# szy4017/DeepSense6G_TII

Hardware: AMD Instinct MI355X
Metric: training samples/sec (5-frame seq, bs=12 per GPU) (higher is better)
Workload: dtype f32; 1 GPU; BASELINE configs[2]: full camera+LiDAR+radar+GPS fusion, 5x(3+1+2)x256x256 + 2x2 GPS per sample, bs=12 per GPU, sigmoid focal loss, AdamW, train-mode BN, dropout 0.1; global_batch=12, seq_len=5, parallelism=dp1, ema=False, launch=eager, optimizer=AdamW after backward

## Files before the change

deepsense6g_tii_amd/csrc/igemm.hip:

```cpp
#include "common.h"
#include "gemm_plan.h"
#include <vector>

extern int g_ds6g_attn_fused128;
extern int g_ds6g_attn_merged_sum;
extern int g_ds6g_attn_percu;
extern int g_ds6g_attn_handover;
extern int g_wino_kb64;

#ifndef IGEMM_STAGES_FD
#define IGEMM_STAGES_FD 3
#endif
#ifndef IGEMM_STAGES_W
#define IGEMM_STAGES_W 2
#endif

GCLK_STORAGE(g_igemm_clk, g_igemm_wg, ds6g_igemm_clocks_read)

namespace {

enum { MODE_FWD = 0, MODE_DGRAD = 1, MODE_WGRAD = 2 };

struct IgemmParams {
    const float* a_src;
    const float* b_src;
    float* out;
    int N, H, W, C;
    int Ho, Wo, K;
    int R, S, stride, pad;
    int Mg, Ng, Kg;
    const float* bias;
    const float* residual;
    const float* mask_src;
    int relu;
    int accumulate;
    uint32_t drop_thr;
    float drop_scale;
    uint64_t seed;
    uint64_t seed_off;
    const uint64_t* salt;
    int k_per_split;
    size_t split_stride;
    int tiles_n;
    int nclass;
    double prof_flops;
    int wg_rows;
    int is_linear;
    int want_colsum;
    int xcd_splits;
    int h0, hstep, Hs, w0, wstep, Ws, r0, rstep, nr, s0, sstep, ns;
    unsigned a_bytes, b_bytes;
    int dbg;
};


template <int MODE, int BM, int BN, int EPI, int BK, int BF, int FAST>
__global__ __launch_bounds__(256) void igemm_kernel(const IgemmParams pin) {
    IgemmParams p = pin;
    if (EPI && p.drop_thr && p.salt) p.seed_off += *p.salt;
    GCLK_DECL(g_igemm_wg);
    if (MODE == MODE_DGRAD && pin.nclass > 1) {
        const int ph = blockIdx.y >> 1, pw = blockIdx.y & 1;
        p.h0 = ph;
        p.w0 = pw;
        p.r0 = (ph + p.pad) & 1;
        p.nr = p.r0 < p.R ? (p.R - p.r0 + 1) / 2 : 0;
        p.s0 = (pw + p.pad) & 1;
        p.ns = p.s0 < p.S ? (p.S - p.s0 + 1) / 2 : 0;
        p.Kg = p.nr * p.ns * p.K;
        if (p.ns == 0) p.ns = 1;
        if (p.Kg == 0 && p.accumulate) return;
    }
    constexpr int CH = BK / 4;
    constexpr int RPB = 16 / CH;
    constexpr int KH = BK / 2;
    constexpr int TM = BM / 64;
    constexpr int TN = BN / 64;
    constexpr int A_LD = BM * CH / 256;
    constexpr int B_LD = BN * CH / 256;
    constexpr bool A_KMAJOR = (MODE == MODE_WGRAD);
    constexpr bool B_KMAJOR = (MODE != MODE_FWD);
    __shared__ __attribute__((aligned(16))) float As0[BM * BK];
    __shared__ __attribute__((aligned(16))) float As1[BM * BK];
    __shared__ __attribute__((aligned(16))) float Bs0[BN * BK];
    __shared__ __attribute__((aligned(16))) float Bs1[BN * BK];
    constexpr int NS = (MODE == MODE_WGRAD) ? IGEMM_STAGES_W : (BK == 32 ? 2 : IGEMM_STAGES_FD);
    static_assert(NS >= 2 && NS <= 4, "2..4 LDS stages");
    __shared__ __attribute__((aligned(16))) float As2[NS >= 3 ? BM * BK : 4];
    __shared__ __attribute__((aligned(16))) float Bs2[NS >= 3 ? BN * BK : 4];
    __shared__ __attribute__((aligned(16))) float As3[NS >= 4 ? BM * BK : 4];
    __shared__ __attribute__((aligned(16))) float Bs3[NS >= 4 ? BN * BK : 4];

    const int tid = threadIdx.x;
    const int lane = tid & 63;
    const int wave = __builtin_amdgcn_readfirstlane(tid >> 6);
    const int wm = wave >> 1, wn = wave & 1;
    int wg, split = blockIdx.z;
    if (MODE == MODE_WGRAD && p.xcd_splits) {
        const int nwg = gridDim.x * gridDim.z, orig = blockIdx.x + gridDim.x * blockIdx.z;
        const int q = nwg >> 3, r = nwg & 7, xcd = orig & 7;
        const int lin = (xcd < r ? xcd * (q + 1) : r * (q + 1) + (xcd - r) * q) + (orig >> 3);
        split = lin / (int)gridDim.x;
        wg = lin - split * (int)gridDim.x;
    } else {
        const int nwg = gridDim.x, orig = blockIdx.x;
        const int q = nwg >> 3, r = nwg & 7, xcd = orig & 7;
        wg = (xcd < r ? xcd * (q + 1) : r * (q + 1) + (xcd - r) * q) + (orig >> 3);
    }
    const int tile_m = wg / p.tiles_n;
    const int tile_n = wg - tile_m * p.tiles_n;
    const int m0 = tile_m * BM, n0 = tile_n * BN;
    const int kbegin = (MODE == MODE_WGRAD) ? split * p.k_per_split : 0;
    const int kend = (MODE == MODE_WGRAD) ? min(p.Kg, kbegin + p.k_per_split) : p.Kg;
    const int nk = (kend - kbegin + BK - 1) / BK;

    const i32x4 a_rsrc = make_srd(p.a_src, p.a_bytes);
    const i32x4 b_rsrc = make_srd(p.b_src, p.b_bytes);

    unsigned a_base[A_LD];
    int a_y[A_LD], a_x[A_LD];
    int a_c[A_LD], a_r[A_LD], a_s[A_LD], a_k[A_LD];
    bool a_ok[A_LD];
#pragma unroll
    for (int i = 0; i < A_LD; ++i) {
        const int idx = tid + i * 256;
        if (MODE == MODE_FWD || MODE == MODE_DGRAD) {
            const int row = idx / CH;
            const int m = m0 + row;
            a_ok[i] = m < p.Mg;
            const int mm = a_ok[i] ? m : 0;
            const int cin = (MODE == MODE_FWD) ? p.C : p.K;
            const int kg = ((idx % CH) ^ ((row / RPB) & (CH - 1))) * 4;
            a_k[i] = kg;
            const int tap = kg / cin;
            a_c[i] = kg - tap * cin;
            const int nsx = (MODE == MODE_DGRAD) ? p.ns : p.S;
            a_r[i] = tap / nsx;
            a_s[i] = tap - a_r[i] * nsx;
            if (MODE == MODE_FWD) {
                int ow, t, oh, n;
                fast_divmod(mm, p.Wo, t, ow);
                fast_divmod(t, p.Ho, n, oh);
                a_y[i] = oh * p.stride - p.pad;
                a_x[i] = ow * p.stride - p.pad;
                a_base[i] = (unsigned)n * (unsigned)(p.H * p.W * p.C);
            } else {
                int ww, t, hh, n;
                fast_divmod(mm, p.Ws, t, ww);
                fast_divmod(t, p.Hs, n, hh);
                a_y[i] = p.h0 + hh * p.hstep + p.pad;
                a_x[i] = p.w0 + ww * p.wstep + p.pad;
                a_base[i] = (unsigned)n * (unsigned)(p.Ho * p.Wo * p.K);
            }
        } else {
            const int mc = idx % (BM / 4);
            a_ok[i] = (m0 + mc * 4) < p.Mg;
            a_k[i] = kbegin + idx / (BM / 4);
            a_base[i] = (unsigned)(m0 + mc * 4);
            a_y[i] = a_x[i] = a_c[i] = a_r[i] = a_s[i] = 0;
        }
    }
    unsigned b_base[B_LD];
    int b_r[B_LD], b_s[B_LD];
    int b_k[B_LD];
    int b_o[B_LD], b_t[B_LD];
    int b_n[B_LD];
    bool b_ok[B_LD];
#pragma unroll
    for (int i = 0; i < B_LD; ++i) {
        const int idx = tid + i * 256;
        b_r[i] = b_s[i] = b_o[i] = b_t[i] = b_n[i] = 0;
        if (MODE == MODE_FWD) {
            const int row = idx / CH;
            b_ok[i] = (n0 + row) < p.Ng;
            b_k[i] = ((idx % CH) ^ ((row / RPB) & (CH - 1))) * 4;
            b_base[i] = (unsigned)(n0 + row) * (unsigned)p.Kg;
        } else if (MODE == MODE_DGRAD) {
            b_ok[i] = (n0 + (idx % (BN / 4)) * 4) < p.Ng;
            const int kg = idx / (BN / 4);
            b_k[i] = kg;
            const int tap = kg / p.K;
            b_o[i] = kg - tap * p.K;
            b_t[i] = tap / p.ns;
            b_n[i] = tap - b_t[i] * p.ns;
            b_base[i] = (unsigned)(n0 + (idx % (BN / 4)) * 4);
        } else {
            const int ncol = n0 + (idx % (BN / 4)) * 4;
            b_ok[i] = ncol < p.Ng;
            const int nn = b_ok[i] ? ncol : 0;
            const int tap = nn / p.C;
            b_r[i] = tap / p.S;
            b_s[i] = tap - b_r[i] * p.S;
            b_base[i] = (unsigned)(nn - tap * p.C);
            const int pix = kbegin + idx / (BN / 4);
            b_k[i] = pix;
            const int pp = pix < p.Kg ? pix : 0;
            b_o[i] = pp % p.Wo;
            const int t = pp / p.Wo;
            b_t[i] = t % p.Ho;
            b_n[i] = t / p.Ho;
        }
    }

    [[maybe_unused]] int u_c0 = 0, u_r = 0, u_s = 0;
    [[maybe_unused]] unsigned u_kb = 0;
    [[maybe_unused]] int u_kpos = kbegin, u_n = 0, u_oh = 0, u_ow = 0;
    [[maybe_unused]] unsigned a_vo[A_LD], b_vo[B_LD];
    [[maybe_unused]] int a_kr[A_LD], b_kr[B_LD], b_ihl[B_LD], b_iwl[B_LD];
    [[maybe_unused]] i32x4 b_rsrc_f = b_rsrc;
    auto retap = [&]() {
#pragma unroll
        for (int i = 0; i < A_LD; ++i) {
            if (MODE == MODE_FWD) {
                const int ih = a_y[i] + u_r, iw = a_x[i] + u_s;
                const bool ok = a_ok[i] && (unsigned)ih < (unsigned)p.H && (unsigned)iw < (unsigned)p.W;
                a_vo[i] = ok ? (a_base[i] + (unsigned)((ih * p.W + iw) * p.C + a_c[i])) * 4u : OOB_OFF;
            } else if (MODE == MODE_DGRAD) {
                const int th = a_y[i] - (p.r0 + u_r * p.rstep), tw = a_x[i] - (p.s0 + u_s * p.sstep);
                int oh = th, ow = tw;
                bool okk = th >= 0 && tw >= 0;
                if (p.stride == 2) {
                    oh = th >> 1;
                    ow = tw >> 1;
                    okk = okk && !((th | tw) & 1);
                } else if (p.stride != 1) {
                    oh = th / p.stride;
                    ow = tw / p.stride;
                    okk = okk && (oh * p.stride == th) && (ow * p.stride == tw);
                }
                const bool ok = a_ok[i] && okk && oh < p.Ho && ow < p.Wo;
                a_vo[i] = ok ? (a_base[i] + (unsigned)((oh * p.Wo + ow) * p.K + a_c[i])) * 4u : OOB_OFF;
            }
        }
    };
    if (FAST) {
        if (MODE == MODE_FWD) {
            retap();
#pragma unroll
            for (int i = 0; i < B_LD; ++i) b_vo[i] = b_ok[i] ? (b_base[i] + (unsigned)b_k[i]) * 4u : OOB_OFF;
        } else if (MODE == MODE_DGRAD) {
            retap();
#pragma unroll
            for (int i = 0; i < B_LD; ++i)
                b_vo[i] = b_ok[i] ? (b_base[i] + (unsigned)(b_o[i] * (p.R * p.S) * p.C)) * 4u : OOB_OFF;
        } else {
            if (p.wg_rows == 0) {
                u_ow = kbegin % p.Wo;
                const int t = kbegin / p.Wo;
                u_oh = t % p.Ho;
                u_n = t / p.Ho;
            } else {
                const int t = kbegin / p.Wo;
                u_oh = t % p.Ho;
                u_n = t / p.Ho;
            }
            const int shift = (p.pad * p.W + p.pad) * p.C;
            b_rsrc_f = make_srd(p.b_src - shift, p.b_bytes + (unsigned)shift * 4u);
#pragma unroll
            for (int i = 0; i < A_LD; ++i) {
                a_kr[i] = (tid + i * 256) / (BM / 4);
                a_vo[i] = (a_base[i] + (unsigned)(a_kr[i] * p.K)) * 4u;
            }
#pragma unroll
            for (int i = 0; i < B_LD; ++i) {
                b_kr[i] = (tid + i * 256) / (BN / 4);
                const int dl_oh = p.wg_rows == 0 ? 0 : b_kr[i] / p.Wo;
                const int dl_ow = p.wg_rows == 0 ? b_kr[i] : b_kr[i] % p.Wo;
                b_ihl[i] = dl_oh * p.stride - p.pad + b_r[i];
                b_iwl[i] = dl_ow * p.stride - p.pad + b_s[i];
                b_vo[i] = (unsigned)((int)b_base[i] + (b_ihl[i] * p.W + b_iwl[i]) * p.C + shift) * 4u;
            }
        }
    }

    auto issue_tiles = [&](float* Ad, float* Bd) {
        if (FAST) {
            if (MODE == MODE_FWD || MODE == MODE_DGRAD) {
                const unsigned sa = (unsigned)u_c0 * 4u;
                unsigned sb;
                if (MODE == MODE_FWD) {
                    sb = u_kb;
                } else {
                    const int tapw = (p.r0 + u_r * p.rstep) * p.S + p.s0 + u_s * p.sstep;
                    sb = (unsigned)((u_c0 * (p.R * p.S) + tapw) * p.C) * 4u;
                }
#pragma unroll
                for (int i = 0; i < A_LD; ++i)
                    dma16(a_rsrc, lds_addr(Ad) + (unsigned)(i * 256 + wave * 64) * 16u, (p.dbg & 32) ? OOB_OFF : a_vo[i], sa);
#pragma unroll
                for (int i = 0; i < B_LD; ++i)
                    dma16(b_rsrc, lds_addr(Bd) + (unsigned)(i * 256 + wave * 64) * 16u, (p.dbg & 32) ? OOB_OFF : b_vo[i], sb);
                u_kb += BK * 4;
                u_c0 += BK;
                if (u_c0 == ((MODE == MODE_FWD) ? p.C : p.K)) {
                    u_c0 = 0;
                    if (++u_s == ((MODE == MODE_FWD) ? p.S : p.ns)) { u_s = 0; ++u_r; }
                    retap();
                }
            } else {
                const int rows_left = kend - u_kpos;
                const unsigned sa = (unsigned)(u_kpos * p.K) * 4u;
                const int ihu = u_oh * p.stride, iwu = u_ow * p.stride;
                const unsigned sb = (unsigned)(((u_n * p.H + ihu) * p.W + iwu) * p.C) * 4u;
#pragma unroll
                for (int i = 0; i < A_LD; ++i) {
                    const bool ok = a_ok[i] && a_kr[i] < rows_left && !(p.dbg & 32);
                    dma16(a_rsrc, lds_addr(Ad) + (unsigned)(i * 256 + wave * 64) * 16u, ok ? a_vo[i] : OOB_OFF, sa);
                }
#pragma unroll
                for (int i = 0; i < B_LD; ++i) {
                    const bool ok = b_ok[i] && b_kr[i] < rows_left && (unsigned)(ihu + b_ihl[i]) < (unsigned)p.H &&
                                    (unsigned)(iwu + b_iwl[i]) < (unsigned)p.W && !(p.dbg & 32);
                    dma16(b_rsrc_f, lds_addr(Bd) + (unsigned)(i * 256 + wave * 64) * 16u, ok ? b_vo[i] : OOB_OFF, sb);
                }
                u_kpos += BK;
                if (p.wg_rows == 0) {
                    u_ow += BK;
                    if (u_ow >= p.Wo) {
                        u_ow = 0;
                        if (++u_oh == p.Ho) { u_oh = 0; ++u_n; }
                    }
                } else {
                    u_oh += p.wg_rows;
                    if (u_oh >= p.Ho) { u_oh = 0; ++u_n; }
                }
            }
            return;
        }
#pragma unroll
        for (int i = 0; i < A_LD; ++i) {
            unsigned off;
            bool ok = a_ok[i] && a_k[i] < kend;
            if (MODE == MODE_FWD) {
                const int ih = a_y[i] + a_r[i], iw = a_x[i] + a_s[i];
                ok = ok && ih >= 0 && ih < p.H && iw >= 0 && iw < p.W;
                off = a_base[i] + (unsigned)((ih * p.W + iw) * p.C + a_c[i]);
            } else if (MODE == MODE_DGRAD) {
                const int th = a_y[i] - (p.r0 + a_r[i] * p.rstep), tw = a_x[i] - (p.s0 + a_s[i] * p.sstep);
                int oh = th, ow = tw;
                bool okk = th >= 0 && tw >= 0;
                if (p.stride == 2) {
                    oh = th >> 1;
                    ow = tw >> 1;
                    okk = okk && !((th | tw) & 1);
                } else if (p.stride != 1) {
                    oh = th / p.stride;
                    ow = tw / p.stride;
                    okk = okk && (oh * p.stride == th) && (ow * p.stride == tw);
                }
                ok = ok && okk && oh < p.Ho && ow < p.Wo;
                off = a_base[i] + (unsigned)((oh * p.Wo + ow) * p.K + a_c[i]);
            } else {
                off = a_base[i] + (unsigned)a_k[i] * (unsigned)p.K;
            }
            if (p.dbg & 32) ok = false;
            dma16(a_rsrc, lds_addr(Ad) + (unsigned)(i * 256 + wave * 64) * 16u, ok ? off * 4u : OOB_OFF, 0u);
            a_k[i] += BK;
            if (MODE != MODE_WGRAD) {
                const int cin = (MODE == MODE_FWD) ? p.C : p.K;
                a_c[i] += BK;
                const int nsx = (MODE == MODE_DGRAD) ? p.ns : p.S;
                while (a_c[i] >= cin) {
                    a_c[i] -= cin;
                    if (++a_s[i] == nsx) { a_s[i] = 0; ++a_r[i]; }
                }
            }
        }
#pragma unroll
        for (int i = 0; i < B_LD; ++i) {
            unsigned off;
            bool ok = b_ok[i] && b_k[i] < kend;
            if (MODE == MODE_FWD) {
                off = b_base[i] + (unsigned)b_k[i];
            } else if (MODE == MODE_DGRAD) {
                const int tap = (p.r0 + b_t[i] * p.rstep) * p.S + p.s0 + b_n[i] * p.sstep;
                off = b_base[i] + (unsigned)((b_o[i] * (p.R * p.S) + tap) * p.C);
                b_o[i] += BK;
                while (b_o[i] >= p.K) {
                    b_o[i] -= p.K;
                    if (++b_n[i] == p.ns) { b_n[i] = 0; ++b_t[i]; }
                }
            } else {
                const int ih = b_t[i] * p.stride - p.pad + b_r[i];
                const int iw = b_o[i] * p.stride - p.pad + b_s[i];
                ok = ok && ih >= 0 && ih < p.H && iw >= 0 && iw < p.W;
                off = b_base[i] + (unsigned)(((b_n[i] * p.H + ih) * p.W + iw) * p.C);
                b_o[i] += BK;
                while (b_o[i] >= p.Wo) {
                    b_o[i] -= p.Wo;
                    if (++b_t[i] == p.Ho) { b_t[i] = 0; ++b_n[i]; }
                }
            }
            if (p.dbg & 32) ok = false;
            dma16(b_rsrc, lds_addr(Bd) + (unsigned)(i * 256 + wave * 64) * 16u, ok ? off * 4u : OOB_OFF, 0u);
            b_k[i] += BK;
        }
    };

    f32x16 acc[TM][TN];
#pragma unroll
    for (int i = 0; i < TM; ++i)
#pragma unroll
        for (int j = 0; j < TN; ++j)
#pragma unroll
            for (int r = 0; r < 16; ++r) acc[i][j][r] = 0.f;

    const int a_row = wm * (BM / 2) + (lane & 31);
    const int b_row = wn * (BN / 2) + (lane & 31);
    const int khalf = lane >> 5;
    const int swz = ((lane & 31) / RPB) & (CH - 1);

    float csum = 0.f;
    const bool do_csum = (MODE == MODE_WGRAD) && p.want_colsum && tile_n == 0 && tid < BM;
    auto k_step = [&](const float* Ac, const float* Bc, float* An, float* Bn, int rem) {
        if (NS >= 3) {
            if (NS >= 4 && rem >= 2) asm volatile("s_waitcnt vmcnt(%0)" ::"n"(2 * (A_LD + B_LD)) : "memory");
            else if (rem >= 1) asm volatile("s_waitcnt vmcnt(%0)" ::"n"(A_LD + B_LD) : "memory");
            else asm volatile("s_waitcnt vmcnt(0)" ::: "memory");
            GCLK(g_igemm_clk, 4);
            if (!(p.dbg & 4)) __syncthreads();
            GCLK(g_igemm_clk, 5);
        }
        if (rem >= NS - 1 && !(p.dbg & 1)) issue_tiles(An, Bn);
        GCLK(g_igemm_clk, 2);
        if (MODE == MODE_WGRAD && do_csum) {
#pragma unroll
            for (int k = 0; k < BK; ++k) csum += Ac[k * BM + tid];
        }
        float af[TM][KH], bf[TN][KH];
#pragma unroll
        for (int i = 0; i < TM; ++i) {
            if (A_KMAJOR) {
#pragma unroll
                for (int kk = 0; kk < KH; ++kk) af[i][kk] = Ac[(khalf * KH + kk) * BM + a_row + i * 32];
            } else {
                const float* rp = &Ac[(a_row + i * 32) * BK];
#pragma unroll
                for (int c = 0; c < CH / 2; ++c) {
                    const f32x4 v = *reinterpret_cast<const f32x4*>(rp + (((khalf * (CH / 2) + c) ^ swz) << 2));
#pragma unroll
                    for (int e = 0; e < 4; ++e) af[i][4 * c + e] = v[e];
                }
            }
        }
#pragma unroll
        for (int j = 0; j < TN; ++j) {
            if (B_KMAJOR) {
#pragma unroll
                for (int kk = 0; kk < KH; ++kk) bf[j][kk] = Bc[(khalf * KH + kk) * BN + b_row + j * 32];
            } else {
                const float* rp = &Bc[(b_row + j * 32) * BK];
#pragma unroll
                for (int c = 0; c < CH / 2; ++c) {
                    const f32x4 v = *reinterpret_cast<const f32x4*>(rp + (((khalf * (CH / 2) + c) ^ swz) << 2));
#pragma unroll
                    for (int e = 0; e < 4; ++e) bf[j][4 * c + e] = v[e];
                }
            }
        }
        __builtin_amdgcn_sched_barrier(0);
        if (BF) {
            static_assert(!BF || BK % 16 == 0, "bf16 k-tiles are multiples of 16");
#pragma unroll
            for (int q = 0; q < BK / 16; ++q) {
                if (BF == 3) {
                    bf16x8 ah[TM], am[TM], al3[TM], bh[TN], bm[TN], bl3[TN];
#pragma unroll
                    for (int i = 0; i < TM; ++i) split3_bf16x8(&af[i][8 * q], ah[i], am[i], al3[i]);
#pragma unroll
                    for (int j = 0; j < TN; ++j) split3_bf16x8(&bf[j][8 * q], bh[j], bm[j], bl3[j]);
#pragma unroll
                    for (int i = 0; i < TM; ++i)
#pragma unroll
                        for (int j = 0; j < TN; ++j)
                            acc[i][j] = mfma_x6(ah[i], am[i], al3[i], bh[j], bm[j], bl3[j], acc[i][j]);
                    continue;
                }
                bf16x8 a8[TM], b8[TN], al[TM], bl[TN];
#pragma unroll
                for (int i = 0; i < TM; ++i) {
                    if (BF == 2) split_bf16x8(&af[i][8 * q], a8[i], al[i]);
                    else {
#pragma unroll
                        for (int e = 0; e < 8; ++e) a8[i][e] = (__bf16)af[i][8 * q + e];
                    }
                }
#pragma unroll
                for (int j = 0; j < TN; ++j) {
                    if (BF == 2) split_bf16x8(&bf[j][8 * q], b8[j], bl[j]);
                    else {
#pragma unroll
                        for (int e = 0; e < 8; ++e) b8[j][e] = (__bf16)bf[j][8 * q + e];
                    }
                }
                if (BF == 2) {
#pragma unroll
                    for (int i = 0; i < TM; ++i)
#pragma unroll
                        for (int j = 0; j < TN; ++j)
                            acc[i][j] = __builtin_amdgcn_mfma_f32_32x32x16_bf16(al[i], b8[j], acc[i][j], 0, 0, 0);
#pragma unroll
                    for (int i = 0; i < TM; ++i)
#pragma unroll
                        for (int j = 0; j < TN; ++j)
                            acc[i][j] = __builtin_amdgcn_mfma_f32_32x32x16_bf16(a8[i], bl[j], acc[i][j], 0, 0, 0);
                }
#pragma unroll
                for (int i = 0; i < TM; ++i)
#pragma unroll
                    for (int j = 0; j < TN; ++j)
                        acc[i][j] = __builtin_amdgcn_mfma_f32_32x32x16_bf16(a8[i], b8[j], acc[i][j], 0, 0, 0);
            }
        } else {
#pragma unroll
            for (int kk = 0; kk < BK / 2; ++kk) {
#pragma unroll
                for (int i = 0; i < TM; ++i)
#pragma unroll
                    for (int j = 0; j < TN; ++j)
                        acc[i][j] = __builtin_amdgcn_mfma_f32_32x32x2f32(af[i][kk], bf[j][kk], acc[i][j], 0, 0, 0);
            }
        }
        __builtin_amdgcn_sched_barrier(0);
        GCLK(g_igemm_clk, 3);
        GCLK_COUNT(g_igemm_clk, 15);
        if (NS == 2) {
            asm volatile("s_waitcnt vmcnt(0)" ::: "memory");
            GCLK(g_igemm_clk, 4);
            if (!(p.dbg & 4)) __syncthreads();
            GCLK(g_igemm_clk, 5);
        }
    };

    float* const Ast[4] = {As0, As1, As2, As3};
    float* const Bst[4] = {Bs0, Bs1, Bs2, Bs3};
    [[maybe_unused]] float bias_pre[TN];
    if (EPI) {
#pragma unroll
        for (int j = 0; j < TN; ++j) {
            const int col = n0 + wn * (BN / 2) + j * 32 + (lane & 31);
            bias_pre[j] = (p.bias && col < p.Ng) ? p.bias[col] : 0.f;
        }
    }
    GCLK(g_igemm_clk, 0);
#pragma unroll
    for (int u = 0; u < NS - 1; ++u)
        if (u < nk && !(p.dbg & 16)) issue_tiles(Ast[u], Bst[u]);
    if (NS == 2) {
        asm volatile("s_waitcnt vmcnt(0)" ::: "memory");
        __syncthreads();
    }
    GCLK(g_igemm_clk, 1);
    for (int kt0 = 0; kt0 < nk; kt0 += NS) {
#pragma unroll
        for (int u = 0; u < NS; ++u) {
            const int kt = kt0 + u;
            if (kt < nk) k_step(Ast[u], Bst[u], Ast[(u + NS - 1) % NS], Bst[(u + NS - 1) % NS], nk - 1 - kt);
        }
    }

    float* outp = p.out + ((MODE == MODE_WGRAD) ? (size_t)split * p.split_stride : (size_t)0);
    if (MODE == MODE_WGRAD && do_csum && m0 + tid < p.Mg) outp[(size_t)p.Mg * p.Ng + m0 + tid] = csum;
    if (EPI == 0) {
        const auto o_rsrc = __builtin_amdgcn_make_buffer_rsrc(outp, 0, (unsigned)p.Mg * (unsigned)p.Ng * 4u, 0x00020000);
        const unsigned rowbytes = (unsigned)p.Ng * 4u;
#pragma unroll
        for (int i = 0; i < TM; ++i) {
#pragma unroll
            for (int j = 0; j < TN; ++j) {
                const int col = n0 + wn * (BN / 2) + j * 32 + (lane & 31);
                const int row0 = m0 + wm * (BM / 2) + i * 32 + 4 * khalf;
                const unsigned base = (col < p.Ng && !((p.dbg & 8) && (i | j)))
                                          ? (unsigned)row0 * rowbytes + (unsigned)col * 4u
                                          : OOB_OFF;
#pragma unroll
                for (int r = 0; r < 16; ++r) {
                    const unsigned off = base + (unsigned)((r & 3) + 8 * (r >> 2)) * rowbytes;
                    float v = acc[i][j][r];
                    if (MODE != MODE_WGRAD && p.accumulate)
                        v += __uint_as_float(__builtin_amdgcn_raw_buffer_load_b32(o_rsrc, off, 0, 0));
                    __builtin_amdgcn_raw_buffer_store_b32(__float_as_uint(v), o_rsrc, off, 0, 0);
                }
            }
        }
        GCLK(g_igemm_clk, 6);
        GCLK_END(g_igemm_clk, g_igemm_wg);
        return;
    }
    if (!(MODE == MODE_DGRAD && p.hstep != 1)) {
        const unsigned nbytes = (unsigned)p.Mg * (unsigned)p.Ng * 4u;
        const auto o_rsrc = __builtin_amdgcn_make_buffer_rsrc(outp, 0, nbytes, 0x00020000);
        const auto m_rsrc = __builtin_amdgcn_make_buffer_rsrc(const_cast<float*>(p.mask_src ? p.mask_src : outp), 0, nbytes, 0x00020000);
        const auto r_rsrc = __builtin_amdgcn_make_buffer_rsrc(const_cast<float*>(p.residual ? p.residual : outp), 0, nbytes, 0x00020000);
        const unsigned rowbytes = (unsigned)p.Ng * 4u;
#pragma unroll
        for (int i = 0; i < TM; ++i) {
#pragma unroll
            for (int j = 0; j < TN; ++j) {
                const int col = n0 + wn * (BN / 2) + j * 32 + (lane & 31);
                const int row0 = m0 + wm * (BM / 2) + i * 32 + 4 * khalf;
                const bool cok = col < p.Ng;
                const float bias = bias_pre[j];
                const unsigned base = cok ? (unsigned)row0 * rowbytes + (unsigned)col * 4u : OOB_OFF;
                const unsigned e0 = (unsigned)row0 * (unsigned)p.Ng + (unsigned)col;
#pragma unroll
                for (int r = 0; r < 16; ++r) {
                    const unsigned dr = (unsigned)((r & 3) + 8 * (r >> 2));
                    const unsigned off = base + dr * rowbytes;
                    float v = acc[i][j][r] + bias;
                    if (p.relu == 1) v = fmaxf(v, 0.f);
                    if (p.mask_src) v = (__uint_as_float(__builtin_amdgcn_raw_buffer_load_b32(m_rsrc, off, 0, 0)) > 0.f) ? v : 0.f;
                    if (p.drop_thr)
                        v = ds6g_keep(p.seed, p.seed_off + (uint64_t)(e0 + dr * (unsigned)p.Ng), p.drop_thr) ? v * p.drop_scale : 0.f;
                    if (p.residual) v += __uint_as_float(__builtin_amdgcn_raw_buffer_load_b32(r_rsrc, off, 0, 0));
                    if (p.accumulate) v += __uint_as_float(__builtin_amdgcn_raw_buffer_load_b32(o_rsrc, off, 0, 0));
                    if (p.relu == 2) v = fmaxf(v, 0.f);
                    __builtin_amdgcn_raw_buffer_store_b32(__float_as_uint(v), o_rsrc, off, 0, 0);
                }
            }
        }
        GCLK(g_igemm_clk, 6);
        GCLK_END(g_igemm_clk, g_igemm_wg);
        return;
    }
#pragma unroll
    for (int i = 0; i < TM; ++i) {
#pragma unroll
        for (int j = 0; j < TN; ++j) {
            const int col = n0 + wn * (BN / 2) + j * 32 + (lane & 31);
            if (col >= p.Ng) continue;
#pragma unroll
            for (int r = 0; r < 16; ++r) {
                const int row = m0 + wm * (BM / 2) + i * 32 + (r & 3) + 8 * (r >> 2) + 4 * khalf;
                if (row >= p.Mg) continue;
                const int ww = row % p.Ws;
                const int t = row / p.Ws;
                const int hh = t % p.Hs;
                const size_t orow = ((size_t)(t / p.Hs) * p.H + p.h0 + hh * p.hstep) * p.W + p.w0 + ww * p.wstep;
                const size_t o = orow * p.Ng + col;
                float v = acc[i][j][r];
                if (p.accumulate) v += outp[o];
                outp[o] = v;
            }
        }
    }
    GCLK(g_igemm_clk, 6);
    GCLK_END(g_igemm_clk, g_igemm_wg);
}

constexpr int RED_COLS = 16, RED_LANES = 16;
__global__ __launch_bounds__(256) void splitk_reduce_kernel(const float* __restrict__ part, float* __restrict__ out,
                                                            long n4, float* __restrict__ out_b, long m4, int splits,
                                                            size_t stride, int accumulate, int accumulate_b) {
    __shared__ f32x4 red[RED_LANES][RED_COLS];
    const int col = threadIdx.x & (RED_COLS - 1), sl = threadIdx.x / RED_COLS;
    const long i = (long)blockIdx.x * RED_COLS + col;
    f32x4 s = {0.f, 0.f, 0.f, 0.f};
    if (i < n4 + m4)
        for (int k = sl; k < splits; k += RED_LANES) s += *reinterpret_cast<const f32x4*>(part + (size_t)k * stride + i * 4);
    red[sl][col] = s;
    __syncthreads();
    if (sl != 0 || i >= n4 + m4) return;
#pragma unroll
    for (int l = 1; l < RED_LANES; ++l) s += red[l][col];
    const bool is_b = i >= n4;
    f32x4* o = is_b ? reinterpret_cast<f32x4*>(out_b + (i - n4) * 4) : reinterpret_cast<f32x4*>(out + i * 4);
    if (is_b ? accumulate_b : accumulate) s += *o;
    *o = s;
}

static_assert(GEMM_ERR_ARG == DS6G_ERR_ARG && GEMM_ERR_WORKSPACE == DS6G_ERR_WORKSPACE && GEMM_OOB == OOB_OFF, "gemm_plan.h");

int g_last_variant = -1;

struct ProfRec { int variant; double flops; hipEvent_t e0, e1; };
std::vector<ProfRec>* g_prof = nullptr;
size_t g_prof_cap = 0;

GemmKnobs g_knobs;
GemmKnobs igemm_knobs() {
    static const bool env_read = [] {
        gemm_env("DS6G_WGRAD_TARGET_LIN", &g_knobs.wgrad_target_lin);
        gemm_env("DS6G_WGRAD_TARGET_CONV", &g_knobs.wgrad_target_conv);
        gemm_env("DS6G_WGRAD_XCD", &g_knobs.wgrad_xcd);
        return true;
    }();
    (void)env_read;
    GemmKnobs kn = g_knobs;
    kn.operand_mode = g_ds6g_bf16;
    return kn;
}

}

void* ds6g_prof_open(int variant, double flops, hipStream_t st) {
    if (!g_prof || g_prof->size() >= g_prof_cap) return nullptr;
    g_prof->push_back(ProfRec{});
    ProfRec* rec = &g_prof->back();
    rec->variant = variant;
    rec->flops = flops;
    (void)hipEventCreate(&rec->e0);
    (void)hipEventCreate(&rec->e1);
    (void)hipEventRecord(rec->e0, st);
    return rec;
}
void ds6g_prof_close(void* rec, hipStream_t st) {
    if (rec) (void)hipEventRecord(static_cast<ProfRec*>(rec)->e1, st);
}

int ds6g_internal_splitk_reduce(const float* ws, float* dw, long n4, float* dbias, long m4, int splits, size_t stride,
                                int accumulate, int accumulate_b, hipStream_t st) {
    hipLaunchKernelGGL(splitk_reduce_kernel, dim3(cdiv(n4 + m4, RED_COLS)), dim3(256), 0, st, ws, dw, n4, dbias, m4, splits,
                       stride, accumulate, accumulate_b);
    DS6G_LAUNCH_CHECK();
    return DS6G_OK;
}

GemmKnobs ds6g_internal_bgemm_knobs();

namespace {

int plan_params(const GemmProblem& q, GemmPlan& pl, IgemmParams& p) {
    if (const int rc = gemm_plan_params(q, igemm_knobs(), pl, p)) return rc;
    p.is_linear = q.op >= DS6G_GEMM_LINEAR_FWD && q.op <= DS6G_GEMM_LINEAR_WGRAD;
    if (pl.nclass > 1) p.prof_flops = 2.0 * p.Mg * p.Ng * (double)(p.R * p.S) * p.K;
    p.dbg = g_knobs.dbg;
    return DS6G_OK;
}

template <int MODE, int CODE>
void launch_igemm(const IgemmParams& p, const GemmPlan& pl, hipStream_t st) {
    constexpr int BF = CODE % 4, KW = CODE / 4 % 3, EPI = CODE / 12 % 2, TILE = CODE / 24;
    constexpr int BM = TILE == 2 ? 64 : 128, BN = TILE == 0 ? 128 : 64;
    if constexpr (!(MODE == MODE_WGRAD && KW == 2))
        hipLaunchKernelGGL((igemm_kernel<MODE, BM, BN, EPI, KW == 2 ? 32 : 16, BF, KW != 0>), dim3(pl.grid_x, pl.grid_y, pl.grid_z),
                           dim3(256), 0, st, p);
}

int run_igemm(const IgemmParams& p, const GemmPlan& pl, float* dw, float* dbias, int accumulate, hipStream_t st) {
    void* rec = ds6g_prof_open(pl.variant, p.prof_flops > 0 ? p.prof_flops : 2.0 * p.Mg * p.Ng * p.Kg, st);
    const int code = ((pl.tile * 2 + pl.epilogue) * 3 + (pl.bk == 32 ? 2 : pl.walk)) * 4 + pl.operand_mode;
    const auto codes = std::make_integer_sequence<int, 3 * 2 * 3 * 4>{};
    if (pl.mode == MODE_FWD) gemm_dispatch(code, [&](auto c) { launch_igemm<MODE_FWD, decltype(c)::value>(p, pl, st); }, codes);
    else if (pl.mode == MODE_DGRAD) gemm_dispatch(code, [&](auto c) { launch_igemm<MODE_DGRAD, decltype(c)::value>(p, pl, st); }, codes);
    else gemm_dispatch(code, [&](auto c) { launch_igemm<MODE_WGRAD, decltype(c)::value>(p, pl, st); }, codes);
    ds6g_prof_close(rec, st);
    g_last_variant = pl.variant;
    DS6G_LAUNCH_CHECK();
    if (!pl.reduce) return DS6G_OK;
    return ds6g_internal_splitk_reduce(p.out, dw, (long)pl.Mg * pl.Ng / 4, dbias, pl.want_colsum ? pl.Mg / 4 : 0, pl.splits,
                                       pl.slab_elems, accumulate, accumulate, st);
}

constexpr int F32 = DS6G_GEMM_F32;

}

extern "C" {

int ds6g_last_igemm_variant(void) { return g_last_variant; }

int ds6g_profile_begin(int max_records) {
    if (max_records <= 0) return DS6G_ERR_ARG;
    if (!g_prof) g_prof = new std::vector<ProfRec>();
    for (auto& r : *g_prof) { (void)hipEventDestroy(r.e0); (void)hipEventDestroy(r.e1); }
    g_prof->clear();
    g_prof->reserve((size_t)max_records);
    g_prof_cap = (size_t)max_records;
    return DS6G_OK;
}

int ds6g_profile_end(int* variants, double* flops, float* ms, int cap) {
    if (!g_prof) return 0;
    int n = 0;
    for (auto& r : *g_prof) {
        (void)hipEventSynchronize(r.e1);
        float t = 0.f;
        (void)hipEventElapsedTime(&t, r.e0, r.e1);
        if (n < cap && variants && flops && ms) { variants[n] = r.variant; flops[n] = r.flops; ms[n] = t; ++n; }
        (void)hipEventDestroy(r.e0);
        (void)hipEventDestroy(r.e1);
    }
    g_prof->clear();
    g_prof_cap = 0;
    return n;
}

int ds6g_set_debug_flags(int flags) {
    g_knobs.dbg = flags & 0xbf;
    g_ds6g_attn_handover = (flags & 0x01000000) ? 0 : 1;
    g_ds6g_attn_fused128 = (flags & 0x04000000) ? 0 : 1;
    g_ds6g_attn_merged_sum = (flags & 0x08000000) ? 0 : 1;
    g_ds6g_attn_percu = (flags >> 20) & 0xf;
    g_wino_kb64 = (flags & 0x02000000) ? 1 : 0;
    g_knobs.bf16_bk32 = (flags & 0x10000000) ? 0 : 1;
    g_knobs.f32_bk32 = (flags & 0x20000000) ? 1 : ((flags & 0x40000000) ? 0 : 2);
    g_knobs.wgrad_tile = (flags & 0x40) ? 2 : 1;
    if ((flags >> 8) & 0xfff) g_knobs.min_blocks = (flags >> 8) & 0xfff;
    return 0;
}

int ds6g_gemm_plan(int family, int op, int N, int H, int W, int C, int K, int R, int S, int stride, int pad, int flags,
                   size_t ws_bytes, struct ds6g_gemm_plan* plan) {
    const GemmProblem q = {family, op, N, H, W, C, K, R, S, stride, pad, (flags & DS6G_GEMM_EPILOGUE) != 0,
                           (flags & DS6G_GEMM_OUT16) != 0, (flags & DS6G_GEMM_ACCUMULATE) != 0, (flags & DS6G_GEMM_DBIAS) != 0, ws_bytes};
    return gemm_plan(q, family == DS6G_GEMM_H16 ? ds6g_internal_bgemm_knobs() : igemm_knobs(), plan);
}

int ds6g_conv2d_fwd(const float* x, const float* w, float* y, int N, int H, int W, int C, int K, int R,
                    int S, int stride, int pad, void* stream) {
    DS6G_ENTER();
    DS6G_CHECK_ARG(x && w && y);
    const GemmProblem q = {F32, DS6G_GEMM_CONV_FWD, N, H, W, C, K, R, S, stride, pad, 0, 0, 0, 0, 0};
    GemmPlan pl; IgemmParams p;
    if (const int rc = plan_params(q, pl, p)) return rc;
    p.a_src = x; p.b_src = w; p.out = y;
    return run_igemm(p, pl, nullptr, nullptr, 0, (hipStream_t)stream);
}

int ds6g_conv2d_dgrad(const float* dy, const float* w, float* dx, int N, int H, int W, int C, int K, int R,
                      int S, int stride, int pad, int accumulate, void* stream) {
    DS6G_ENTER();
    DS6G_CHECK_ARG(dy && w && dx);
    const GemmProblem q = {F32, DS6G_GEMM_CONV_DGRAD, N, H, W, C, K, R, S, stride, pad, 0, 0, accumulate, 0, 0};
    GemmPlan pl; IgemmParams p;
    if (const int rc = plan_params(q, pl, p)) return rc;
    p.a_src = dy; p.b_src = w; p.out = dx;
    return run_igemm(p, pl, nullptr, nullptr, 0, (hipStream_t)stream);
}

int ds6g_conv2d_wgrad(const float* x, const float* dy, float* dw, int N, int H, int W, int C, int K, int R,
                      int S, int stride, int pad, int accumulate, float* ws, size_t ws_bytes, void* stream) {
    DS6G_ENTER();
    DS6G_CHECK_ARG(x && dy && dw);
    const GemmProblem q = {F32, DS6G_GEMM_CONV_WGRAD, N, H, W, C, K, R, S, stride, pad, 0, 0, accumulate, 0, ws_bytes};
    GemmPlan pl; IgemmParams p;
    if (const int rc = plan_params(q, pl, p)) return rc;
    DS6G_CHECK_ARG(ws || !pl.reduce);
    p.a_src = dy; p.b_src = x; p.out = pl.reduce ? ws : dw;
    return run_igemm(p, pl, dw, nullptr, accumulate, (hipStream_t)stream);
}

int ds6g_conv2d_bias_act_fwd(const float* x, const float* w, const float* bias, const float* residual, float* y, int N,
                             int H, int W, int C, int K, int R, int S, int stride, int pad, int relu, void* stream) {
    DS6G_ENTER();
    DS6G_CHECK_ARG(x && w && y && relu >= 0 && relu <= 2);
    const GemmProblem q = {F32, DS6G_GEMM_CONV_BIAS_ACT_FWD, N, H, W, C, K, R, S, stride, pad, bias || relu || residual, 0, 0, 0, 0};
    GemmPlan pl; IgemmParams p;
    if (const int rc = plan_params(q, pl, p)) return rc;
    p.a_src = x; p.b_src = w; p.out = y; p.bias = bias; p.residual = residual; p.relu = relu;
    return run_igemm(p, pl, nullptr, nullptr, 0, (hipStream_t)stream);
}

int ds6g_linear_fwd(const float* x, const float* w, const float* bias, float* y, int M, int N, int K, int relu,
                    const float* residual, float drop_p, uint64_t seed, uint64_t seed_off, void* stream) {
    DS6G_ENTER();
    DS6G_CHECK_ARG(x && w && y && drop_p >= 0.f && drop_p < 1.f);
    const uint32_t drop_thr = ds6g_drop_threshold(drop_p);
    const GemmProblem q = {F32, DS6G_GEMM_LINEAR_FWD, 1, 1, M, K, N, 1, 1, 1, 0, bias || relu || drop_thr || residual, 0, 0, 0, 0};
    GemmPlan pl; IgemmParams p;
    if (const int rc = plan_params(q, pl, p)) return rc;
    p.a_src = x; p.b_src = w; p.out = y; p.bias = bias; p.relu = relu; p.residual = residual;
    p.drop_thr = drop_thr;
    p.drop_scale = 1.f / (1.f - drop_p);
    p.seed = seed; p.seed_off = seed_off; p.salt = g_ds6g_salt;
    return run_igemm(p, pl, nullptr, nullptr, 0, (hipStream_t)stream);
}

int ds6g_linear_dgrad(const float* dy, const float* w, float* dx, int M, int N, int K, const float* mask_src,
                      int accumulate, void* stream) {
    DS6G_ENTER();
    DS6G_CHECK_ARG(dy && w && dx);
    const GemmProblem q = {F32, DS6G_GEMM_LINEAR_DGRAD, 1, 1, M, K, N, 1, 1, 1, 0, mask_src != nullptr, 0, accumulate, 0, 0};
    GemmPlan pl; IgemmParams p;
    if (const int rc = plan_params(q, pl, p)) return rc;
    p.a_src = dy; p.b_src = w; p.out = dx; p.mask_src = mask_src;
    return run_igemm(p, pl, nullptr, nullptr, 0, (hipStream_t)stream);
}

int ds6g_linear_wgrad(const float* x, const float* dy, float* dw, float* dbias, int M, int N, int K, int accumulate,
                      float* ws, size_t ws_bytes, void* stream) {
    DS6G_ENTER();
    DS6G_CHECK_ARG(x && dy && dw);
    const GemmProblem q = {F32, DS6G_GEMM_LINEAR_WGRAD, 1, 1, M, K, N, 1, 1, 1, 0, 0, 0, accumulate, dbias != nullptr, ws_bytes};
    GemmPlan pl; IgemmParams p;
    if (const int rc = plan_params(q, pl, p)) return rc;
    DS6G_CHECK_ARG(ws || !pl.reduce);
    p.a_src = dy; p.b_src = x; p.out = pl.reduce ? ws : dw;
    return run_igemm(p, pl, dw, dbias, accumulate, (hipStream_t)stream);
}

}
```

Before: 186.4 samples/s.

## Batch igemm epilogue loads ahead of stores and prefetch epilogue operands before mainloop

Restructures the implicit-GEMM epilogue so the residual, mask and accumulate loads are issued in batches ahead of the stores, with scheduling barriers and compile-time specialisation on which operands are present. For small 1x1 tiles, one epilogue operand is prefetched before the K loop so its latency overlaps the main loop. The strided dgrad scatter path is replaced with incremental index arithmetic and buffer loads and stores, keeping a fallback for tensors too large for 32-bit offsets. The aim is to hide global-memory latency in the store phase, at the cost of extra registers, possible occupancy loss, and larger code from the template variants.

```diff
diff --git a/deepsense6g_tii_amd/csrc/igemm.hip b/deepsense6g_tii_amd/csrc/igemm.hip
--- a/deepsense6g_tii_amd/csrc/igemm.hip
+++ b/deepsense6g_tii_amd/csrc/igemm.hip
@@ -1,5 +1,6 @@
 #include "common.h"
 #include "gemm_plan.h"
+#include <type_traits>
 #include <vector>
 
 extern int g_ds6g_attn_fused128;
@@ -20,6 +21,11 @@
 namespace {
 
 enum { MODE_FWD = 0, MODE_DGRAD = 1, MODE_WGRAD = 2 };
+
+__device__ __forceinline__ unsigned opaque_u32(unsigned x) {
+    asm volatile("" : "+v"(x));
+    return x;
+}
 
 struct IgemmParams {
     const float* a_src;
@@ -542,6 +548,27 @@
             bias_pre[j] = (p.bias && col < p.Ng) ? p.bias[col] : 0.f;
         }
     }
+    constexpr bool EPI_PRE = EPI && MODE != MODE_WGRAD && TM == 1 && TN == 1 && BF == 0 && BK == 16;
+    constexpr int EPI_BATCH = MODE == MODE_WGRAD ? 4 : TM * TN == 2 ? 32 : 16;
+    const int epi_sel = (p.mask_src ? 1 : 0) | (p.residual ? 2 : 0) | (p.accumulate ? 4 : 0);
+    const bool epi_remap = MODE == MODE_DGRAD && p.hstep != 1;
+    auto blk_base = [&](int i, int j) -> unsigned {
+        const int col = n0 + wn * (BN / 2) + j * 32 + (lane & 31);
+        const int row0 = m0 + wm * (BM / 2) + i * 32 + 4 * (lane >> 5);
+        return col < p.Ng ? ((unsigned)row0 * (unsigned)p.Ng + (unsigned)col) * 4u : OOB_OFF;
+    };
+    auto reg_row = [](int f) -> unsigned { return (unsigned)((f & 3) + 8 * ((f >> 2) & 3)); };
+    float* outp = p.out + ((MODE == MODE_WGRAD) ? (size_t)split * p.split_stride : (size_t)0);
+    [[maybe_unused]] float epi_pre[16];
+    if (EPI_PRE) {
+        const float* src = p.mask_src ? p.mask_src : p.residual ? p.residual : outp;
+        const unsigned bytes = (epi_sel && !epi_remap) ? (unsigned)p.Mg * (unsigned)p.Ng * 4u : 0u;
+        const auto rsrc = __builtin_amdgcn_make_buffer_rsrc(const_cast<float*>(src), 0, bytes, 0x00020000);
+        const unsigned base = blk_base(0, 0), rowbytes = (unsigned)p.Ng * 4u;
+#pragma unroll
+        for (int r = 0; r < 16; ++r)
+            epi_pre[r] = __uint_as_float(__builtin_amdgcn_raw_buffer_load_b32(rsrc, base + (unsigned)((r & 3) + 8 * (r >> 2)) * rowbytes, 0, 0));
+    }
     GCLK(g_igemm_clk, 0);
 #pragma unroll
     for (int u = 0; u < NS - 1; ++u)
@@ -559,90 +586,178 @@
         }
     }
 
-    float* outp = p.out + ((MODE == MODE_WGRAD) ? (size_t)split * p.split_stride : (size_t)0);
     if (MODE == MODE_WGRAD && do_csum && m0 + tid < p.Mg) outp[(size_t)p.Mg * p.Ng + m0 + tid] = csum;
+    constexpr int NREG = TM * TN * 16;
     if (EPI == 0) {
         const auto o_rsrc = __builtin_amdgcn_make_buffer_rsrc(outp, 0, (unsigned)p.Mg * (unsigned)p.Ng * 4u, 0x00020000);
         const unsigned rowbytes = (unsigned)p.Ng * 4u;
-#pragma unroll
-        for (int i = 0; i < TM; ++i) {
-#pragma unroll
-            for (int j = 0; j < TN; ++j) {
-                const int col = n0 + wn * (BN / 2) + j * 32 + (lane & 31);
-                const int row0 = m0 + wm * (BM / 2) + i * 32 + 4 * khalf;
-                const unsigned base = (col < p.Ng && !((p.dbg & 8) && (i | j)))
-                                          ? (unsigned)row0 * rowbytes + (unsigned)col * 4u
-                                          : OOB_OFF;
-#pragma unroll
-                for (int r = 0; r < 16; ++r) {
-                    const unsigned off = base + (unsigned)((r & 3) + 8 * (r >> 2)) * rowbytes;
-                    float v = acc[i][j][r];
-                    if (MODE != MODE_WGRAD && p.accumulate)
-                        v += __uint_as_float(__builtin_amdgcn_raw_buffer_load_b32(o_rsrc, off, 0, 0));
-                    __builtin_amdgcn_raw_buffer_store_b32(__float_as_uint(v), o_rsrc, off, 0, 0);
-                }
-            }
-        }
+        unsigned base[TM * TN];
+#pragma unroll
+        for (int b = 0; b < TM * TN; ++b) base[b] = ((p.dbg & 8) && b) ? OOB_OFF : blk_base(b / TN, b % TN);
+        auto store_tiles = [&](auto acc_c) {
+            constexpr bool ACC = decltype(acc_c)::value;
+#pragma unroll
+            for (int f0 = 0; f0 < NREG; f0 += EPI_BATCH) {
+                [[maybe_unused]] float ov[EPI_BATCH];
+                unsigned sbase = 0;
+                __builtin_amdgcn_sched_barrier(0);
+                if (ACC) {
+#pragma unroll
+                    for (int f = f0; f < f0 + EPI_BATCH; ++f)
+                        ov[f - f0] = __uint_as_float(__builtin_amdgcn_raw_buffer_load_b32(o_rsrc, base[f >> 4] + reg_row(f) * rowbytes, 0, 0));
+                    __builtin_amdgcn_sched_barrier(0);
+                }
+#pragma unroll
+                for (int f = f0; f < f0 + EPI_BATCH; ++f) {
+                    if (f == f0 || (f & 15) == 0) sbase = opaque_u32(base[f >> 4]);
+                    float v = acc[(f >> 4) / TN][(f >> 4) % TN][f & 15];
+                    if (ACC) v += ov[f - f0];
+                    __builtin_amdgcn_raw_buffer_store_b32(__float_as_uint(v), o_rsrc, sbase + reg_row(f) * rowbytes, 0, 0);
+                }
+            }
+        };
+        if (MODE != MODE_WGRAD && p.accumulate) store_tiles(std::true_type{});
+        else store_tiles(std::false_type{});
         GCLK(g_igemm_clk, 6);
         GCLK_END(g_igemm_clk, g_igemm_wg);
         return;
     }
-    if (!(MODE == MODE_DGRAD && p.hstep != 1)) {
+    if (!epi_remap) {
         const unsigned nbytes = (unsigned)p.Mg * (unsigned)p.Ng * 4u;
         const auto o_rsrc = __builtin_amdgcn_make_buffer_rsrc(outp, 0, nbytes, 0x00020000);
         const auto m_rsrc = __builtin_amdgcn_make_buffer_rsrc(const_cast<float*>(p.mask_src ? p.mask_src : outp), 0, nbytes, 0x00020000);
         const auto r_rsrc = __builtin_amdgcn_make_buffer_rsrc(const_cast<float*>(p.residual ? p.residual : outp), 0, nbytes, 0x00020000);
         const unsigned rowbytes = (unsigned)p.Ng * 4u;
-#pragma unroll
-        for (int i = 0; i < TM; ++i) {
-#pragma unroll
-            for (int j = 0; j < TN; ++j) {
-                const int col = n0 + wn * (BN / 2) + j * 32 + (lane & 31);
-                const int row0 = m0 + wm * (BM / 2) + i * 32 + 4 * khalf;
-                const bool cok = col < p.Ng;
-                const float bias = bias_pre[j];
-                const unsigned base = cok ? (unsigned)row0 * rowbytes + (unsigned)col * 4u : OOB_OFF;
-                const unsigned e0 = (unsigned)row0 * (unsigned)p.Ng + (unsigned)col;
-#pragma unroll
-                for (int r = 0; r < 16; ++r) {
-                    const unsigned dr = (unsigned)((r & 3) + 8 * (r >> 2));
-                    const unsigned off = base + dr * rowbytes;
-                    float v = acc[i][j][r] + bias;
+        unsigned base[TM * TN], e0[TM * TN];
+#pragma unroll
+        for (int b = 0; b < TM * TN; ++b) {
+            base[b] = blk_base(b / TN, b % TN);
+            e0[b] = (unsigned)(m0 + wm * (BM / 2) + (b / TN) * 32 + 4 * khalf) * (unsigned)p.Ng +
+                    (unsigned)(n0 + wn * (BN / 2) + (b % TN) * 32 + (lane & 31));
+        }
+        auto epi_tiles = [&](auto hm_c, auto hr_c, auto ha_c) {
+            constexpr bool HM = decltype(hm_c)::value, HR = decltype(hr_c)::value, HA = decltype(ha_c)::value;
+            constexpr int PRE = !EPI_PRE ? 0 : HM ? 1 : HR ? 2 : HA ? 3 : 0;
+            constexpr int NLOAD = HM + HR + HA - (PRE ? 1 : 0);
+            constexpr int RB = NLOAD <= 1 ? EPI_BATCH : NLOAD == 2 ? EPI_BATCH / 2 : EPI_BATCH / 4;
+#pragma unroll
+            for (int f0 = 0; f0 < NREG; f0 += RB) {
+                [[maybe_unused]] float mv[RB], rv[RB], ov[RB];
+                unsigned sbase = 0;
+                __builtin_amdgcn_sched_barrier(0);
+#pragma unroll
+                for (int f = f0; f < f0 + RB; ++f) {
+                    const unsigned off = base[f >> 4] + reg_row(f) * rowbytes;
+                    if (HM) mv[f - f0] = PRE == 1 ? epi_pre[f & 15] : __uint_as_float(__builtin_amdgcn_raw_buffer_load_b32(m_rsrc, off, 0, 0));
+                    if (HR) rv[f - f0] = PRE == 2 ? epi_pre[f & 15] : __uint_as_float(__builtin_amdgcn_raw_buffer_load_b32(r_rsrc, off, 0, 0));
+                    if (HA) ov[f - f0] = PRE == 3 ? epi_pre[f & 15] : __uint_as_float(__builtin_amdgcn_raw_buffer_load_b32(o_rsrc, off, 0, 0));
+                }
+                if (NLOAD) __builtin_amdgcn_sched_barrier(0);
+#pragma unroll
+                for (int f = f0; f < f0 + RB; ++f) {
+#pragma clang fp contract(off)
+                    if (f == f0 || (f & 15) == 0) sbase = opaque_u32(base[f >> 4]);
+                    float v = acc[(f >> 4) / TN][(f >> 4) % TN][f & 15] + bias_pre[(f >> 4) % TN];
                     if (p.relu == 1) v = fmaxf(v, 0.f);
-                    if (p.mask_src) v = (__uint_as_float(__builtin_amdgcn_raw_buffer_load_b32(m_rsrc, off, 0, 0)) > 0.f) ? v : 0.f;
+                    if (HM) v = (mv[f - f0] > 0.f) ? v : 0.f;
                     if (p.drop_thr)
-                        v = ds6g_keep(p.seed, p.seed_off + (uint64_t)(e0 + dr * (unsigned)p.Ng), p.drop_thr) ? v * p.drop_scale : 0.f;
-                    if (p.residual) v += __uint_as_float(__builtin_amdgcn_raw_buffer_load_b32(r_rsrc, off, 0, 0));
-                    if (p.accumulate) v += __uint_as_float(__builtin_amdgcn_raw_buffer_load_b32(o_rsrc, off, 0, 0));
+                        v = ds6g_keep(p.seed, p.seed_off + (uint64_t)(e0[f >> 4] + reg_row(f) * (unsigned)p.Ng), p.drop_thr) ? v * p.drop_scale : 0.f;
+                    if (HR) v += rv[f - f0];
+                    if (HA) v += ov[f - f0];
                     if (p.relu == 2) v = fmaxf(v, 0.f);
-                    __builtin_amdgcn_raw_buffer_store_b32(__float_as_uint(v), o_rsrc, off, 0, 0);
-                }
-            }
+                    __builtin_amdgcn_raw_buffer_store_b32(__float_as_uint(v), o_rsrc, sbase + reg_row(f) * rowbytes, 0, 0);
+                }
+            }
+        };
+        const std::true_type T{};
+        const std::false_type F{};
+        switch (epi_sel) {
+            case 0: epi_tiles(F, F, F); break;
+            case 1: epi_tiles(T, F, F); break;
+            case 2: epi_tiles(F, T, F); break;
+            case 3: epi_tiles(T, T, F); break;
+            case 4: epi_tiles(F, F, T); break;
+            case 5: epi_tiles(T, F, T); break;
+            case 6: epi_tiles(F, T, T); break;
+            default: epi_tiles(T, T, T); break;
         }
         GCLK(g_igemm_clk, 6);
         GCLK_END(g_igemm_clk, g_igemm_wg);
         return;
     }
-#pragma unroll
-    for (int i = 0; i < TM; ++i) {
-#pragma unroll
-        for (int j = 0; j < TN; ++j) {
-            const int col = n0 + wn * (BN / 2) + j * 32 + (lane & 31);
-            if (col >= p.Ng) continue;
-#pragma unroll
-            for (int r = 0; r < 16; ++r) {
-                const int row = m0 + wm * (BM / 2) + i * 32 + (r & 3) + 8 * (r >> 2) + 4 * khalf;
-                if (row >= p.Mg) continue;
-                const int ww = row % p.Ws;
-                const int t = row / p.Ws;
-                const int hh = t % p.Hs;
-                const size_t orow = ((size_t)(t / p.Hs) * p.H + p.h0 + hh * p.hstep) * p.W + p.w0 + ww * p.wstep;
-                const size_t o = orow * p.Ng + col;
-                float v = acc[i][j][r];
-                if (p.accumulate) v += outp[o];
-                outp[o] = v;
-            }
-        }
+    constexpr int SG = TM * TN >= 4 ? 1 : 2;
+    const auto s_rsrc = __builtin_amdgcn_make_buffer_rsrc(
+        outp, 0, (unsigned)p.N * (unsigned)p.H * (unsigned)p.W * (unsigned)p.Ng * 4u, 0x00020000);
+    auto scatter_tiles = [&](auto acc_c) {
+        constexpr bool ACC = decltype(acc_c)::value;
+#pragma unroll
+        for (int i = 0; i < TM; ++i) {
+#pragma unroll
+            for (int g0 = 0; g0 < 4; g0 += SG) {
+                unsigned off[TN][4 * SG];
+                [[maybe_unused]] float ov[TN][4 * SG];
+                __builtin_amdgcn_sched_barrier(0);
+#pragma unroll
+                for (int g = g0; g < g0 + SG; ++g) {
+                    const int rg = m0 + wm * (BM / 2) + i * 32 + 8 * g + 4 * khalf;
+                    int ww = rg % p.Ws;
+                    const int t = rg / p.Ws;
+                    int hh = t % p.Hs;
+                    int n = t / p.Hs;
+#pragma unroll
+                    for (int q = 0; q < 4; ++q) {
+                        const unsigned orow = (unsigned)((n * p.H + p.h0 + hh * p.hstep) * p.W + p.w0 + ww * p.wstep);
+#pragma unroll
+                        for (int j = 0; j < TN; ++j) {
+                            const int col = n0 + wn * (BN / 2) + j * 32 + (lane & 31);
+                            const int e = 4 * (g - g0) + q;
+                            off[j][e] = (rg + q < p.Mg && col < p.Ng) ? (orow * (unsigned)p.Ng + (unsigned)col) * 4u : OOB_OFF;
+                            if (ACC) ov[j][e] = __uint_as_float(__builtin_amdgcn_raw_buffer_load_b32(s_rsrc, off[j][e], 0, 0));
+                        }
+                        if (++ww == p.Ws) {
+                            ww = 0;
+                            if (++hh == p.Hs) { hh = 0; ++n; }
+                        }
+                    }
+                }
+#pragma unroll
+                for (int j = 0; j < TN; ++j)
+#pragma unroll
+                    for (int e = 0; e < 4 * SG; ++e) {
+                        float v = acc[i][j][4 * g0 + e];
+                        if (ACC) v += ov[j][e];
+                        __builtin_amdgcn_raw_buffer_store_b32(__float_as_uint(v), s_rsrc, off[j][e], 0, 0);
+                    }
+            }
+        }
+    };
+    const size_t s_bytes = (size_t)p.N * p.H * p.W * p.Ng * 4;
+    if (s_bytes > (size_t)OOB_OFF) {
+#pragma unroll
+        for (int i = 0; i < TM; ++i) {
+#pragma unroll
+            for (int j = 0; j < TN; ++j) {
+                const int col = n0 + wn * (BN / 2) + j * 32 + (lane & 31);
+                if (col >= p.Ng) continue;
+#pragma unroll
+                for (int r = 0; r < 16; ++r) {
+                    const int row = m0 + wm * (BM / 2) + i * 32 + (r & 3) + 8 * (r >> 2) + 4 * khalf;
+                    if (row >= p.Mg) continue;
+                    const int ww = row % p.Ws;
+                    const int t = row / p.Ws;
+                    const int hh = t % p.Hs;
+                    const size_t orow = ((size_t)(t / p.Hs) * p.H + p.h0 + hh * p.hstep) * p.W + p.w0 + ww * p.wstep;
+                    const size_t o = orow * p.Ng + col;
+                    float v = acc[i][j][r];
+                    if (p.accumulate) v += outp[o];
+                    outp[o] = v;
+                }
+            }
+        }
+    } else if (p.accumulate) {
+        scatter_tiles(std::true_type{});
+    } else {
+        scatter_tiles(std::false_type{});
     }
     GCLK(g_igemm_clk, 6);
     GCLK_END(g_igemm_clk, g_igemm_wg);
```

New measurement: 188.3 samples/s, median of 6. +1.0%, better.
